# mlelarge/graph_neural_net

Hardware: AMD Instinct MI355X
Metric: graph-pairs/sec FGNN fwd+bwd, N=50 regular pairs (higher is better)
Workload: dtype f32

## Files before the change

### graph_neural_net_amd/_lib.py

```python
import ctypes as C
import os

import torch

_HERE = os.path.dirname(os.path.abspath(__file__))
LIB_PATH = os.environ.get('FGNN_LIB') or os.path.join(_HERE, 'libfgnn_hip.so')

FGNN_H = 32
FGNN_TILE = 32
FGNN_MAX_DEPTH = 3
FGNN_RANGE_WG = 256
FGNN_LSAP_MAX_N = 2048
FGNN_MAX_LEVELS = 64
FGNN_QAP_MAX_N = 256
FGNN_QAPW_MAX_N = 256
FGNN_SPECTRAL_MAX_N = 256
FGNN_SPECTRAL_MAX_POWERS = 8
FGNN_PLANTED_MAX_N = 256
FGNN_SCORE_SPLIT = 4

c_float_p = C.c_void_p


class Slab(C.Structure):
# ... 62 lines not shown
                ('s12tiles', C.c_void_p), ('s12_out', C.c_void_p), ('xbits', C.c_void_p), ('xdeg', C.c_void_p),
                ('ranges', C.c_void_p), ('cu_share', C.c_int)]


class Slab16(C.Structure):
    _fields_ = [('ptr', C.c_void_p), ('gstride', C.c_longlong), ('ldp', C.c_longlong), ('C', C.c_int),
                ('nrm', C.c_void_p), ('beta', C.c_void_p)]


class MlpFwd16Args(C.Structure):
    _fields_ = [('G', C.c_int), ('N', C.c_int), ('ldr', C.c_int), ('depth', C.c_int), ('nmlp', C.c_int),
                ('nvalid', C.c_void_p),
                ('a', Slab16), ('b', Slab16),
                ('z', C.c_void_p * 2), ('ldz', C.c_longlong),
                ('part', C.c_void_p * 2), ('cnt', C.c_void_p), ('packed', C.c_void_p), ('ranges', C.c_void_p)]


class MlpBwd16Args(C.Structure):
    _fields_ = [('G', C.c_int), ('N', C.c_int), ('ldr', C.c_int), ('depth', C.c_int),
                ('nvalid', C.c_void_p),
                ('a', Slab16), ('b', Slab16),
                ('dy', C.c_void_p), ('dgstride', C.c_longlong), ('ldd', C.c_longlong),
                ('z', C.c_void_p), ('zgstride', C.c_longlong), ('ldz', C.c_longlong),
                ('coef', C.c_void_p),
                ('dxa', C.c_void_p), ('dxa_gstride', C.c_longlong), ('dxa_ld', C.c_longlong),
                ('dxb', C.c_void_p), ('dxb_gstride', C.c_longlong), ('dxb_ld', C.c_longlong),
                ('accumulate_a', C.c_int), ('accumulate_b', C.c_int),
                ('wpart', C.c_void_p), ('s12part', C.c_void_p), ('packed', C.c_void_p), ('ranges', C.c_void_p)]


class GradJob(C.Structure):
    _fields_ = [('wpart', C.c_void_p), ('count', C.c_int), ('out', C.c_void_p), ('s12', C.c_void_p),
                ('nrm', C.c_void_p), ('dgn_w', C.c_void_p), ('dgn_b', C.c_void_p), ('rows', C.c_int), ('scale', C.c_float), ('scale_dev', C.c_void_p)]


class PackJob(C.Structure):
    _fields_ = [('kind', C.c_int), ('ca', C.c_int), ('cb', C.c_int), ('depth', C.c_int), ('nmlp', C.c_int),
                ('W', (C.c_void_p * FGNN_MAX_DEPTH) * 2), ('bias', (C.c_void_p * FGNN_MAX_DEPTH) * 2),
                ('out', C.c_void_p)]


class PairgenArgs(C.Structure):
    _fields_ = [('seed', C.c_ulonglong), ('first', C.c_longlong), ('B', C.c_int), ('N', C.c_int),
                ('family', C.c_int), ('noise_model', C.c_int), ('edge_density', C.c_double),
                ('thr_edge', C.c_ulonglong), ('thr_noise1', C.c_ulonglong), ('thr_noise2', C.c_ulonglong),
                ('thr_vertex', C.c_ulonglong), ('swaps_per_edge', C.c_int),
                ('bits1', C.c_void_p), ('bits2', C.c_void_p), ('nvalid', C.c_void_p)]


FGNN_GUARD_MAX_PARTS = 64
FGNN_GUARD_SKIP_NONFINITE = 1
FGNN_GUARD_NONFINITE = 1


class GuardRecord(C.Structure):
    _fields_ = [('max_norm', C.c_double), ('norm', C.c_double), ('coef', C.c_double),
                ('flags', C.c_int), ('skipped', C.c_int), ('arrivals', C.c_int), ('mode', C.c_int),
                ('partial', C.c_double * FGNN_GUARD_MAX_PARTS)]


class EvalRecord(C.Structure):
    _fields_ = [('ce_sum', C.c_double), ('nodes', C.c_longlong), ('correct_lsap', C.c_longlong), ('correct_max', C.c_longlong),
                ('pairs', C.c_longlong), ('steps', C.c_longlong)]


MAX_GRAD_JOBS = 16
MAX_PACK_JOBS = 24
_VP, _LL, _I, _F = C.c_void_p, C.c_longlong, C.c_int, C.c_float

_SIGNATURES = {
    'fgnn_last_error': [],
    'fgnn_version': [],
    'fgnn_tiles_per_graph': [_I],
    'fgnn_mlp_bwd_num_workgroups': [],
    'fgnn_pack_floats': [_I, _I, _I, _I, _I],
    'fgnn_pack_operands': [_VP, _I, _VP],
    'fgnn_mlp_fwd': [C.POINTER(MlpFwdArgs), _VP],
    'fgnn_pack_x3_floats': [_I, _I, _I, _I, _I],
    'fgnn_pack_x3_operands': [_VP, _I, _VP],
    'fgnn_mlp_fwd_x3': [C.POINTER(MlpFwdArgs), _VP],
    'fgnn_debug_mlp_fwd_masks': [C.POINTER(MlpFwdArgs), _VP, _VP, _VP],
    'fgnn_debug_mlp_fwd_x3_masks': [C.POINTER(MlpFwdArgs), _VP, _VP, _VP],
    'fgnn_debug_matmul_variant': [_I],
    'fgnn_gn_finalize': [_VP, _VP, _VP, _VP, _I, _I, _I, _F, _VP, _VP],
    'fgnn_gn_finalize2': [_VP, _VP, _VP, _VP, _VP, _VP, _I, _I, _I, _F, _VP, _VP, _VP],
    'fgnn_gn_plane_supported': [_I],
    'fgnn_gn_plane_fwd': [_VP, _LL, _LL, _VP, _VP, _VP, _I, _I, _I, _F, _VP, _LL, _LL, _VP, _VP],
    'fgnn_gn_plane_bwd': [_VP, _LL, _LL, _VP, _LL, _LL, _VP, _VP, _I, _I, _I, _VP, _LL, _LL, _VP, _VP, _VP, _VP],
    'fgnn_gn_stats': [_VP, _LL, _LL, _VP, _VP, _I, _I, _I, _F, _VP, _VP],
    'fgnn_gn_apply': [_VP, _LL, _LL, _VP, _VP, _VP, _I, _I, _I, _VP, _LL, _LL, _VP],
    'fgnn_ragged_tile_ranges': [_VP, _I, _I, _VP, _VP],
    'fgnn_ragged_tile_ranges_order': [_VP, _I, _I, _VP, _VP, _VP],
    'fgnn_ragged_tile_ranges16': [_VP, _I, _I, _I, _VP, _VP],
    'fgnn_conv1x1_dw_multi': [C.POINTER(DwJob), _I, _VP, _I, _I, _VP, _VP],
    'fgnn_conv_chain_supported': [_I, _I, C.POINTER(C.c_int)],
    'fgnn_conv_chain': [C.POINTER(ChainArgs), _VP],
    'fgnn_mlp64_supported': [_I, _I, _I],
    'fgnn_mlp64_num_workgroups': [],
    'fgnn_mlp64_param_count': [_I],
    'fgnn_mlp64_packed_floats': [_I],
    'fgnn_mlp64_pack': [_VP, _VP, _VP, _VP, _VP, _VP, _I, _VP, _VP],
    'fgnn_mlp64_pack_multi': [C.POINTER(Mlp64PackJob), _I, _VP],
    'fgnn_mlp64_fwd': [C.POINTER(Mlp64Args), _VP],
    'fgnn_mlp64_bwd': [C.POINTER(Mlp64Args), _VP],
    'fgnn_conv1x1': [_VP, _LL, _LL, _VP, _VP, _LL, _LL, _VP, _I, _VP, _I, _I, _I, _I, _VP, _LL, _LL, _VP],
    'fgnn_conv1x1_dw_chunks': [_I, _I],
    'fgnn_conv1x1_dw': [_VP, _LL, _LL, _VP, _VP, _LL, _LL, _VP, _I, _I, _I, _I, _VP, _VP],
    'fgnn_chan_matmul_fwd': [C.POINTER(Slab), C.POINTER(Slab), _VP, _I, _I, _VP, _LL, _LL, _VP],
    'fgnn_chan_matmul_fwd_ord': [C.POINTER(Slab), C.POINTER(Slab), _VP, _I, _I, _VP, _LL, _LL, _VP, _I, _VP],
    'fgnn_chan_matmul_fwd_fin_supported': [_I],
    'fgnn_chan_matmul_fwd_fin': [C.POINTER(Slab), C.POINTER(Slab), _VP, _VP, _VP, _VP, _VP, _F, _VP, _I, _I, _VP, _LL, _LL, _VP],
    'fgnn_chan_matmul_fwd_fin_ord': [C.POINTER(Slab), C.POINTER(Slab), _VP, _VP, _VP, _VP, _VP, _F, _VP, _I, _I, _VP, _LL, _LL, _VP, _I, _VP],
    'fgnn_colmax_fwd': [C.POINTER(Slab), _VP, _I, _I, _VP, _VP, _VP],
    'fgnn_colmax_fwd_fin_supported': [_I],
    'fgnn_colmax_fwd_fin': [C.POINTER(Slab), _VP, _VP, _VP, _F, _VP, _I, _I, _VP, _VP, _VP],
    'fgnn_score_ce_fwd': [_VP, _VP, _VP, _I, _I, _I, _VP, _VP, _VP, _VP],
    'fgnn_score_row_blocks': [_I, _I],
    'fgnn_score_ce_fwd_blocks': [_VP, _VP, _VP, _I, _I, _I, _I, _VP, _VP, _VP, _VP],
    'fgnn_score_ce_bwd': [_VP, _VP, _VP, _VP, _VP, _VP, _I, _I, _I, _VP, _VP, _VP],
    'fgnn_score_ce_fwd_blocks_labels': [_VP, _VP, _VP, _VP, _I, _I, _I, _I, _VP, _VP, _VP, _VP],
    'fgnn_score_ce_bwd_labels': [_VP, _VP, _VP, _VP, _VP, _VP, _VP, _I, _I, _I, _VP, _VP, _VP],
    'fgnn_ce_fwd_labels': [_VP, _VP, _VP, _I, _I, _VP, _VP, _VP],
    'fgnn_ce_bwd_labels': [_VP, _VP, _VP, _VP, _VP, _I, _I, _VP, _VP],
    'fgnn_inv_node_count': [_VP, _I, _VP, _VP],
    'fgnn_score_bwd': [_VP, _VP, _VP, _VP, _I, _I, _I, _VP, _VP, _VP],
    'fgnn_ce_fwd': [_VP, _VP, _I, _I, _VP, _VP, _VP],
    'fgnn_ce_bwd': [_VP, _VP, _VP, _VP, _I, _I, _VP, _VP],
    'fgnn_colmax_bwd': [_VP, _VP, _VP, _I, _I, _I, _VP, _LL, _LL, C.POINTER(Slab), _VP, _VP],
    'fgnn_gn_bwd_stats': [_VP, _LL, _LL, _VP, _LL, _LL, _VP, _VP, _I, _I, _I, _VP, _VP],
    'fgnn_gn_bwd_coef': [_VP, _VP, _VP, _I, _I, _I, _VP, _VP, _VP, _VP],
    'fgnn_gn_bwd_coef_tiles': [_VP, _VP, _VP, _I, _I, _I, _VP, _VP, _VP],
    'fgnn_grad_finalize': [_VP, _I, _I, _I, _I, _VP],
    'fgnn_gn_bwd_apply': [_VP, _LL, _LL, _VP, _LL, _LL, _VP, _VP, _I, _I, _I, _VP, _LL, _LL, _VP],
    'fgnn_mlp_bwd': [C.POINTER(MlpBwdArgs), _VP],
    'fgnn_mlp_bwd_x3': [C.POINTER(MlpBwdArgs), _VP],
    'fgnn_mlp_bwd_pair': [C.POINTER(MlpBwdArgs), C.POINTER(MlpBwdArgs), _VP],
    'fgnn_mlp_bwd_t16': [C.POINTER(MlpBwdArgs), _VP],
    'fgnn_mlp_bwd_t16_supported': [C.POINTER(MlpBwdArgs)],
    'fgnn_mlp_bwd_pair_t16': [C.POINTER(MlpBwdArgs), C.POINTER(MlpBwdArgs), _VP],
    'fgnn_mlp_bwd_pair_x3': [C.POINTER(MlpBwdArgs), C.POINTER(MlpBwdArgs), _VP],
    'fgnn_block1_struct_supported': [_I, _I, _I],
    'fgnn_block1_struct_table_floats': [_I],
    'fgnn_block1_struct_ws_floats': [_I, _I],
    'fgnn_block1_struct_rows': [_I, _I],
    'fgnn_block1_struct_fwd': [_VP, _VP, _I, _I, _VP, _VP, _VP, _VP, _VP, C.c_float, _VP, _VP, _VP, _LL, _LL, _VP, _VP, _VP, _VP, _VP, _VP, _VP],
    'fgnn_block1_struct_bwd': [_VP, _VP, _I, _I, _VP, _VP, _VP, _VP, _VP, _VP, _VP, _VP, _LL, _LL, _VP, _VP, _VP, _VP, _VP, _VP],
    'fgnn_block1_struct_fwd_pack': [_VP, _VP, _I, _I, _VP, _VP, _VP, _VP, _VP, C.c_float, _VP, _VP, _VP, _LL, _LL, _VP, _VP, _VP, _VP, _VP, _VP, _VP, _I, _VP],
    'fgnn_block1_struct_fwd16_pack': [_VP, _VP, _I, _I, _I, _VP, _VP, _VP, _VP, _VP, C.c_float, _VP, _VP, _VP, _LL, _LL, _VP, _VP, _VP, _VP, _VP, _VP, _VP, _I, _VP],
    'fgnn_block1_struct_fwd16': [_VP, _VP, _I, _I, _I, _VP, _VP, _VP, _VP, _VP, C.c_float, _VP, _VP, _VP, _LL, _LL, _VP, _VP, _VP, _VP, _VP, _VP, _VP],
    'fgnn_block1_struct_bwd16': [_VP, _VP, _I, _I, _I, _VP, _VP, _VP, _VP, _VP, _VP, _VP, _VP, _LL, _LL, _VP, _VP, _VP, _VP, _VP, _VP],
    'fgnn_mlp_bwd_coef_tiles_supported': [_I, _I],
    'fgnn_mlp_param_count': [_I, _I],
    'fgnn_reduce_partials': [_VP, _I, _I, _VP, _VP],
    'fgnn_chan_matmul_bwd': [C.POINTER(Slab), C.POINTER(Slab), _VP, _LL, _LL, _VP, _I, _I, _VP, _VP, _LL, _LL, _VP, _VP, _VP],
    'fgnn_chan_matmul_bwd_ord': [C.POINTER(Slab), C.POINTER(Slab), _VP, _LL, _LL, _VP, _I, _I, _VP, _VP, _LL, _LL, _VP, _VP, _VP, _I, _VP],
    'fgnn_sum_scale': [_VP, _I, _I, _F, _VP, _VP],
    'fgnn_adam_step': [_VP, _VP, _VP, _VP, _I, C.c_double, C.c_double, C.c_double, C.c_double, _I, C.c_double, _VP],
    'fgnn_adam_step_dev': [_VP, _VP, _VP, _VP, _I, _VP, _VP, _VP],
    'fgnn_grad_guard': [_VP, _I, _VP, _VP, _VP],
    'fgnn_adam_step_guarded': [_VP, _VP, _VP, _VP, _I, _VP, _VP, _VP, _VP],
    'fgnn_expand_adjacency': [_VP, _VP, _I, _I, _VP, _VP],
    'fgnn_pack_adjacency': [_VP, _VP, _I, _I, _VP, _VP, _VP],
    'fgnn_pack_adjacency_ld': [_VP, _VP, _I, _I, _I, _VP, _VP, _VP],
    'fgnn_pack_adjacency_pair': [_VP, _VP, _VP, _VP, _I, _I, _I, _VP, _VP, _VP, _VP, _VP],
    'fgnn_adjacency_degree': [_VP, _VP, _I, _I, _VP, _VP],
    'fgnn_accuracy_max': [_VP, _VP, _I, _I, _VP, _VP],
# ... 147 lines not shown
```

### graph_neural_net_amd/csrc/matmul.hip

```cpp
#include "fgnn_common.h"
#include "fgnn_norm.h"

namespace {

constexpr int TM = 64;
constexpr int LDS_LD = 65;

struct NormRec {
    float mean, a, beta;
    bool on;
};

DEVI NormRec norm_of(const fgnn_slab &s, int g, int c) {
    NormRec r;
    r.on = s.nrm != nullptr;
    if (r.on) {
        const float4 n = reinterpret_cast<const float4 *>(s.nrm)[(long long)g * s.C + c];
        r.mean = n.x;
        r.a = n.y;
        r.beta = s.beta ? s.beta[c] : 0.f;
    } else {
        r.mean = 0.f;
        r.a = 1.f;
        r.beta = 0.f;
// ... 121 lines not shown
    if (s12a && live) {
        const int col = col0 + 32 * qj + j;
#pragma unroll
        for (int r = 0; r < 16; ++r) {
            const int row = row0 + 32 * qi + ch_of(r, h);
            if (row < nv && col < nv) {
                sa1 += acc[r];
                sa2 += acc[r] * (A[(long long)row * N + col] - na.mean);
            }
        }
    }

#pragma unroll
    for (int r = 0; r < 16; ++r) acc[r] = 0.f;
    for (int i0 = 0; i0 < N; i0 += TM) {
        __syncthreads();
        stage_tile(Xs, A, N, nv, i0, row0, na, tid);
        stage_tile(Ds, D, N, nv, i0, col0, none, tid);
        __syncthreads();
        if (live) {
            const int kmax = (N - i0 < TM ? N - i0 : TM);
            const float *ap = Xs + h * LDS_LD + 32 * qi + j;
            const float *bp = Ds + h * LDS_LD + 32 * qj + j;
            for (int k = 0; k < kmax; k += 2) acc = mfma32(ap[k * LDS_LD], bp[k * LDS_LD], acc);
        }
    }
    if (live) store_quadrant(OB, N, row0 + 32 * qi, col0 + 32 * qj, acc, lane);
    if (s12a) {
        if (live) {
            const int col = col0 + 32 * qj + j;
#pragma unroll
            for (int r = 0; r < 16; ++r) {
                const int row = row0 + 32 * qi + ch_of(r, h);
                if (row < nv && col < nv) {
                    sb1 += acc[r];
                    sb2 += acc[r] * (B[(long long)row * N + col] - nb.mean);
                }
            }
        }
        sa1 = wave_sum(sa1);
        sa2 = wave_sum(sa2);
        sb1 = wave_sum(sb1);
        sb2 = wave_sum(sb2);
        if (lane == 0) {
            red[wave][0] = sa1;
            red[wave][1] = sa2;
            red[wave][2] = sb1;
            red[wave][3] = sb2;
        }
        __syncthreads();
        if (tid < 4) {
            const float v = (red[0][tid] + red[1][tid]) + (red[2][tid] + red[3][tid]);
            float *dst = (tid < 2 ? s12a : s12b) + (long long)gc * 2 + (tid & 1);
            *dst = v;
        }
    }
}

template <bool WANT_U>
DEVI void load_tile_regs(float (&v)[16], float (&u)[16], const float *mat, int N, int nv, const NormRec &nr, int tid) {
#pragma unroll
    for (int k = 0; k < 16; ++k) {
        const int e = tid + 256 * k;
        const int r = e >> 6, c = e & 63;
        const bool ok = r < nv && c < nv;
        const float x = mat[ok ? r * N + c : 0];
        const float d = x - nr.mean;
        v[k] = ok ? (nr.on ? d * nr.a + nr.beta : x) : 0.f;
        if (WANT_U) u[k] = ok ? d : 0.f;
    }
}
DEVI void store_tile_lds(float *lds, const float (&v)[16], int tid) {
#pragma unroll
    for (int k = 0; k < 16; ++k) {
        const int e = tid + 256 * k;
        lds[(e >> 6) * LDS_LD + (e & 63)] = v[k];
    }
}
DEVI void frag_to_lds(float *lds, int row0, int col0, const f32x16 &acc, int lane) {
    const int j = lane & 31, h = lane >> 5;
#pragma unroll
    for (int r = 0; r < 16; ++r) lds[(row0 + ch_of(r, h)) * LDS_LD + col0 + j] = acc[r];
}
template <bool WANT_S>
DEVI void tile_to_global(const View &ov, int mat_off4, const float *lds, int N, const float (&u)[16], float &s1,
                         float &s2, int tid) {
    const int c = tid & 63, r0 = __builtin_amdgcn_readfirstlane(tid >> 6);
    const int voff = c < N ? (r0 * N + c) * 4 : OOB_OFF;
    const float *lp = lds + r0 * LDS_LD + c;
#pragma unroll
    for (int k = 0; k < 16; ++k) {
        const float t = lp[4 * k * LDS_LD];
        buf_store(t, ov, r0 + 4 * k < N ? voff : OOB_OFF, mat_off4 + k * 16 * N);
        if (WANT_S) {
            s1 += t;
            s2 += t * u[k];
        }
    }
}

DEVI void load_tile_raw(float (&x)[16], const View &v, int mat_off4, int N, int nv, int tid) {
    const int c = tid & 63, r0 = __builtin_amdgcn_readfirstlane(tid >> 6);
    const int voff = c < nv ? (r0 * N + c) * 4 : OOB_OFF;
#pragma unroll
    for (int k = 0; k < 16; ++k) {
        const int r = r0 + 4 * k;
        x[k] = buf_load(v, r < nv ? voff : OOB_OFF, mat_off4 + k * 16 * N);
    }
}
template <bool WANT_U>
DEVI void finish_tile(float (&v)[16], float (&u)[16], const float (&x)[16], int nv, const NormRec &nr, int tid) {
#pragma unroll
    for (int k = 0; k < 16; ++k) {
        const int e = tid + 256 * k;
        const int r = e >> 6, c = e & 63;
        const bool ok = r < nv && c < nv;
        const float d = x[k] - nr.mean;
        v[k] = ok ? (nr.on ? d * nr.a + nr.beta : x[k]) : 0.f;
        if (WANT_U) u[k] = ok ? d : 0.f;
    }
}

struct FinArgs {
    const float *part_a, *part_b, *cnt, *gw_a, *gw_b;
    float *nrm_a, *nrm_b;
    float eps;
    int tpg;
};
template <bool FIN>
__global__ __launch_bounds__(256, 4) void chan_matmul_fwd1_kernel(const fgnn_slab ya, const fgnn_slab yb,
                                                               const int *nvalid, int N, int M, float *out,
                                                               long long ogstride, long long ldo, const FinArgs F) {
    __shared__ float As[TM * LDS_LD];
    __shared__ float Bs[TM * LDS_LD];
    __shared__ float4 fin_rec[2];
    const int C = ya.C;
    const int tid = threadIdx.x, lane = tid & 63, wave = tid >> 6;
    const int qi = wave >> 1, qj = wave & 1;
    const int j = lane & 31, h = lane >> 5;
    float xa[16], xb[16], dummy[16];
    const int G = M / C;
    const View vA = make_view(ya.ptr, ya.gstride, ya.ldp, G), vB = make_view(yb.ptr, yb.gstride, yb.ldp, G);
    const View vO = make_view(out, ogstride, ldo, G);
    const int gc = blockIdx.x;
    {
        const int g = gc / C, c = gc - g * C;
        const int nv = nvalid_of(nvalid, g, N);
        TilePartials tp;
        if (FIN && wave < 2) tp = finalize_load(wave ? F.part_b : F.part_a, F.cnt, g, c, C, F.tpg, lane);
        load_tile_raw(xa, vA, g * vA.gs4 + c * vA.ld4, N, nv, tid);
        load_tile_raw(xb, vB, g * vB.gs4 + c * vB.ld4, N, nv, tid);
        NormRec na, nb;
        if (FIN) {
            if (wave < 2) {
                const float4 r = finalize_reduce(tp, (float)nv, (wave ? F.gw_b : F.gw_a) ? (wave ? F.gw_b : F.gw_a)[c] : 1.f, F.eps);
                if (lane == 0) {
                    fin_rec[wave] = r;
                    reinterpret_cast<float4 *>(wave ? F.nrm_b : F.nrm_a)[gc] = r;
                }
            }
            __syncthreads();
            const float4 ra = fin_rec[0], rb = fin_rec[1];
            na.on = true; na.mean = ra.x; na.a = ra.y; na.beta = ya.beta ? ya.beta[c] : 0.f;
            nb.on = true; nb.mean = rb.x; nb.a = rb.y; nb.beta = yb.beta ? yb.beta[c] : 0.f;
        } else {
            na = norm_of(ya, g, c);
            nb = norm_of(yb, g, c);
        }
        const int o_off = g * vO.gs4 + c * vO.ld4;
        {
            float va[16], vb[16];
            finish_tile<false>(va, dummy, xa, nv, na, tid);
            finish_tile<false>(vb, dummy, xb, nv, nb, tid);
            store_tile_lds(As, va, tid);
            store_tile_lds(Bs, vb, tid);
// ... 24 lines not shown
    __shared__ float Ds[TM * LDS_LD];
    __shared__ float red[4][4];
    const int C = ya.C;
    const int tid = threadIdx.x, lane = tid & 63, wave = tid >> 6;
    const int qi = wave >> 1, qj = wave & 1;
    const int j = lane & 31, h = lane >> 5;
    NormRec none;
    none.on = false; none.mean = 0.f; none.a = 1.f; none.beta = 0.f;
    float xa[16], xb[16], xd[16], dummy[16];
    const int G = M / C;
    const View vA = make_view(ya.ptr, ya.gstride, ya.ldp, G), vB = make_view(yb.ptr, yb.gstride, yb.ldp, G);
    const View vD = make_view(dm, dmg, ldm, G);
    const View vOA = make_view(da, ogstride, ldo, G), vOB = make_view(db, ogstride, ldo, G);
    const int gc = blockIdx.x;
    {
        const int g = gc / C, c = gc - g * C;
        const int nv = nvalid_of(nvalid, g, N);
        load_tile_raw(xa, vA, g * vA.gs4 + c * vA.ld4, N, nv, tid);
        load_tile_raw(xb, vB, g * vB.gs4 + c * vB.ld4, N, nv, tid);
        load_tile_raw(xd, vD, g * vD.gs4 + c * vD.ld4, N, nv, tid);
        const NormRec na = norm_of(ya, g, c), nb = norm_of(yb, g, c);
        const int o_off = g * vOA.gs4 + c * vOA.ld4;
        float ua[16], ub[16], va[16];
        finish_tile<true>(va, ua, xa, nv, na, tid);
        {
            float vb[16], vd[16];
            finish_tile<true>(vb, ub, xb, nv, nb, tid);
            finish_tile<false>(vd, dummy, xd, nv, none, tid);
            store_tile_lds(Bs, vb, tid);
            store_tile_lds(Ds, vd, tid);
        }
        __syncthreads();
        const bool live = 32 * qi < N && 32 * qj < N;
        f32x16 accA, accB;
#pragma unroll
        for (int r = 0; r < 16; ++r) {
            accA[r] = 0.f;
            accB[r] = 0.f;
        }
        if (live) {
            const float *ap = Ds + (32 * qi + j) * LDS_LD + h;
            const float *bp = Bs + (32 * qj + j) * LDS_LD + h;
            for (int k = 0; k < N; k += 2) accA = mfma32(ap[k], bp[k], accA);
        }
        __syncthreads();
        store_tile_lds(Bs, va, tid);
        __syncthreads();
        if (live) {
            const float *ap = Bs + h * LDS_LD + 32 * qi + j;
            const float *bp = Ds + h * LDS_LD + 32 * qj + j;
            for (int k = 0; k < N; k += 2) accB = mfma32(ap[k * LDS_LD], bp[k * LDS_LD], accB);
        }
        __syncthreads();
        frag_to_lds(Ds, 32 * qi, 32 * qj, accA, lane);
        frag_to_lds(Bs, 32 * qi, 32 * qj, accB, lane);
        __syncthreads();
        float sa1 = 0.f, sa2 = 0.f, sb1 = 0.f, sb2 = 0.f;
        if (s12a) {
            tile_to_global<true>(vOA, o_off, Ds, N, ua, sa1, sa2, tid);
            tile_to_global<true>(vOB, o_off, Bs, N, ub, sb1, sb2, tid);
            sa1 = wave_sum(sa1);
            sa2 = wave_sum(sa2);
            sb1 = wave_sum(sb1);
            sb2 = wave_sum(sb2);
            if (lane == 0) {
                red[wave][0] = sa1;
                red[wave][1] = sa2;
                red[wave][2] = sb1;
                red[wave][3] = sb2;
            }
            __syncthreads();
            if (tid < 4) {
                const float v = (red[0][tid] + red[1][tid]) + (red[2][tid] + red[3][tid]);
                float *dst = (tid < 2 ? s12a : s12b) + (long long)gc * 2 + (tid & 1);
                *dst = v;
            }
        } else {
            tile_to_global<false>(vOA, o_off, Ds, N, dummy, sa1, sa2, tid);
            tile_to_global<false>(vOB, o_off, Bs, N, dummy, sb1, sb2, tid);
        }
    }
}


int g_mm_wave_variant = 1;
inline bool mm_wave_variant() { return (g_mm_wave_variant & 1) != 0; }
inline bool mm_narrow() { return (g_mm_wave_variant & 8) != 0; }
constexpr int WLD = 68;
constexpr int W_WAVES = 2;

DEVI rsrc_t mat_rsrc(const float *p, int bytes) {
    return __builtin_amdgcn_make_buffer_rsrc(const_cast<float *>(p), 0, bytes, 0x00020000);
}
DEVI float rsrc_load(rsrc_t r, int voff, int soff) {
    return __builtin_bit_cast(float, __builtin_amdgcn_raw_buffer_load_b32(r, voff, soff, 0));
}
DEVI void rsrc_store(float x, rsrc_t r, int voff, int soff) {
    __builtin_amdgcn_raw_buffer_store_b32(__builtin_bit_cast(unsigned, x), r, voff, soff, 0);
}

template <int KQ>
DEVI void wave_rows_load(float (&x)[8 * KQ], rsrc_t r, int N, int voff) {
#pragma unroll
    for (int i = 0; i < 8 * KQ; ++i) x[i] = rsrc_load(r, voff, i < N ? i * N * 4 : 0);
}
template <int KQ>
DEVI void wave_rows_stage(float *T, const float (&x)[8 * KQ], float mean, float a_eff, float b_eff, int nv, int N, int lane) {
    if (nv < N) {
#pragma unroll
        for (int i = 0; i < 8 * KQ; ++i) {
            const float v = (x[i] - mean) * a_eff + b_eff;
            T[i * WLD + lane] = i < nv ? v : 0.f;
        }
    } else {
#pragma unroll
        for (int i = 0; i < 8 * KQ; ++i) T[i * WLD + lane] = (x[i] - mean) * a_eff + b_eff;
    }
}

template <int KQ, bool FIN>
__global__ __launch_bounds__(64 * W_WAVES, 2) void chan_matmul_fwd_w_kernel(const fgnn_slab ya, const fgnn_slab yb,
                                                                           const int *nvalid, int N, int M, float *out,
                                                                           long long ogstride, long long ldo,
                                                                           const FinArgs F) {
    constexpr int KH = 4 * KQ;
    constexpr bool TWO = KQ > 4;
    constexpr int NB = TWO ? 2 : 1;
    __shared__ __attribute__((aligned(16))) float lds[W_WAVES * 32 * NB * WLD];
    const int lane = threadIdx.x & 63, wv = __builtin_amdgcn_readfirstlane(threadIdx.x >> 6);
    const int gc = xcd_swizzle(blockIdx.x, gridDim.x) * W_WAVES + wv;
    if (gc >= M) return;
    const int C = ya.C;
    const int g = gc / C, c = gc - g * C;
    const int nv = __builtin_amdgcn_readfirstlane(nvalid_of(nvalid, g, N));
    const int j = lane & 31, h = lane >> 5;
    float *As = lds + wv * (32 * NB * WLD);
    const rsrc_t rA = mat_rsrc(ya.ptr + (long long)g * ya.gstride + (long long)c * ya.ldp, nv * N * 4);
    const rsrc_t rB = mat_rsrc(yb.ptr + (long long)g * yb.gstride + (long long)c * yb.ldp, nv * N * 4);
    const rsrc_t rO = mat_rsrc(out + (long long)g * ogstride + (long long)c * ldo, N * N * 4);

    TilePartials ta, tb;
    if (FIN) {
        ta = finalize_load(F.part_a, F.cnt, g, c, C, F.tpg, lane);
        tb = finalize_load(F.part_b, F.cnt, g, c, C, F.tpg, lane);
    }
    float xa[8 * KQ], xb[NB][KH];
    wave_rows_load<KQ>(xa, rA, N, lane < nv ? lane * 4 : OOB_OFF);
    int voffB[NB];
#pragma unroll
    for (int cb = 0; cb < NB; ++cb) {
        const int col = 32 * cb + j;
        voffB[cb] = col < nv ? (h * N + col) * 4 : OOB_OFF;
    }
#pragma unroll
    for (int s = 0; s < KH; ++s)
#pragma unroll
        for (int cb = 0; cb < NB; ++cb) xb[cb][s] = rsrc_load(rB, voffB[cb] + s * 2 * N * 4, 0);
    float meanA, aA, meanB, aB;
    if (FIN) {
        const float4 ra = finalize_reduce(ta, (float)nv, F.gw_a ? F.gw_a[c] : 1.f, F.eps);
        const float4 rb = finalize_reduce(tb, (float)nv, F.gw_b ? F.gw_b[c] : 1.f, F.eps);
        if (lane == 0) {
            reinterpret_cast<float4 *>(F.nrm_a)[gc] = ra;
            reinterpret_cast<float4 *>(F.nrm_b)[gc] = rb;
        }
        meanA = ra.x; aA = ra.y; meanB = rb.x; aB = rb.y;
    } else {
        const NormRec na = norm_of(ya, g, c), nb = norm_of(yb, g, c);
// ... 518 lines not shown
        sa2 = wave_sum(sa2);
        sb1 = wave_sum(sb1);
        sb2 = wave_sum(sb2);
        if (lane == 0) {
            red[wv][0] = sa1;
            red[wv][1] = sa2;
            red[wv][2] = sb1;
            red[wv][3] = sb2;
        }
        __syncthreads();
        if (tid < 4 && (tid < 2 ? do_a : do_b)) {
            float v = 0.f;
#pragma unroll
            for (int w = 0; w < BIG_NW; ++w) v += red[w][tid];
            float *dst = (tid < 2 ? s12a : s12b) + (long long)gc * 2 + (tid & 1);
            *dst = v;
        }
    }
}

inline bool big_path(int N) { return N > TM && N <= 256; }

}

template <int MT, bool FIN>
static void launch_fwd_big(const fgnn_slab *ya, const fgnn_slab *yb, const int *nvalid, int N, int G, float *out, long long ogstride,
                           long long ldo, const int *order, const FinArgs &F, int fill, hipStream_t st) {
    static LdsAttrCache attr_cache;
    (void)fgnn_raise_lds(attr_cache, (const void *)chan_matmul_fwd_big_kernel<MT, FIN>, BigCfg<MT>::LDS_BYTES);
    hipLaunchKernelGGL((chan_matmul_fwd_big_kernel<MT, FIN>), dim3(G * ya->C), dim3(BIG_THREADS), BigCfg<MT>::LDS_BYTES, st, *ya, *yb, nvalid, N, G, out,
                       ogstride, ldo, order, F, fill);
}

extern "C" int fgnn_chan_matmul_fwd(const fgnn_slab *ya, const fgnn_slab *yb, const int *nvalid, int G, int N,
                                    float *out, long long ogstride, long long ldo, void *stream) {
    return fgnn_chan_matmul_fwd_ord(ya, yb, nvalid, G, N, out, ogstride, ldo, nullptr, 0, stream);
}

extern "C" int fgnn_chan_matmul_fwd_ord(const fgnn_slab *ya, const fgnn_slab *yb, const int *nvalid, int G, int N,
                                        float *out, long long ogstride, long long ldo, const int *order, int fill, void *stream) {
    FGNN_CHECK(!order || nvalid, "fgnn_chan_matmul_fwd_ord: an order needs the nvalid it was derived from");
    FGNN_CHECK(ya && yb && out && ya->ptr && yb->ptr, "fgnn_chan_matmul_fwd: null argument");
    FGNN_CHECK(ya->C == yb->C && ya->C > 0 && G > 0 && N > 0, "fgnn_chan_matmul_fwd: bad shapes");
    FGNN_CHECK((long long)G * ya->C <= 65535 * 1024ll, "fgnn_chan_matmul_fwd: G*C too large");
    const int t = (N + TM - 1) / TM;
    if (t == 1) {
        FGNN_CHECK((long long)G * ya->gstride < 0x7fffffffll / 4 && (long long)G * yb->gstride < 0x7fffffffll / 4,
                   "fgnn_chan_matmul_fwd: a tensor exceeds 2 GiB (32-bit buffer addressing); split the batch");
        FGNN_CHECK((long long)G * ogstride < 0x7fffffffll / 4, "fgnn_chan_matmul_fwd: output exceeds 2 GiB");
        const int M = G * ya->C;
        if (mm_wave_variant()) {
            launch_fwd_w<false>(ya, yb, nvalid, N, M, out, ogstride, ldo, FinArgs{}, (hipStream_t)stream);
            FGNN_LAUNCH_CHECK();
            return 0;
        }
        hipLaunchKernelGGL(chan_matmul_fwd1_kernel<false>, dim3(M), dim3(256), 0, (hipStream_t)stream, *ya, *yb, nvalid,
                           N, M, out, ogstride, ldo, FinArgs{});
        FGNN_LAUNCH_CHECK();
        return 0;
    }
    if (big_path(N)) {
        FGNN_CHECK((long long)G * ya->gstride < 0x7fffffffll / 4 && (long long)G * yb->gstride < 0x7fffffffll / 4 &&
                   (long long)G * ogstride < 0x7fffffffll / 4,
                   "fgnn_chan_matmul_fwd: a tensor exceeds 2 GiB (32-bit buffer addressing); split the batch");
        if (N <= 128) launch_fwd_big<4, false>(ya, yb, nvalid, N, G, out, ogstride, ldo, order, FinArgs{}, fill, (hipStream_t)stream);
        else launch_fwd_big<8, false>(ya, yb, nvalid, N, G, out, ogstride, ldo, order, FinArgs{}, fill, (hipStream_t)stream);
        FGNN_LAUNCH_CHECK();
        return 0;
    }
    hipLaunchKernelGGL(chan_matmul_fwd_kernel, dim3(t, t, G * ya->C), dim3(256), 0, (hipStream_t)stream, *ya, *yb,
                       nvalid, N, out, ogstride, ldo);
    FGNN_LAUNCH_CHECK();
    return 0;
}

extern "C" int fgnn_chan_matmul_fwd_fin_supported(int N) { return (N <= TM || big_path(N)) ? 1 : 0; }

extern "C" int fgnn_debug_matmul_variant(int wave_per_matrix) {
    FGNN_CHECK((wave_per_matrix & ~9) == 0, "fgnn_debug_matmul_variant: bits 0 and 3 only (got %d)", wave_per_matrix);
    g_mm_wave_variant = wave_per_matrix;
    return 0;
}

extern "C" int fgnn_chan_matmul_fwd_fin(const fgnn_slab *ya, const fgnn_slab *yb, const float *part_a, const float *part_b,
                                        const float *cnt, const float *gn_weight_a, const float *gn_weight_b, float eps,
                                        const int *nvalid, int G, int N, float *out, long long ogstride, long long ldo,
                                        void *stream) {
    return fgnn_chan_matmul_fwd_fin_ord(ya, yb, part_a, part_b, cnt, gn_weight_a, gn_weight_b, eps, nvalid, G, N, out, ogstride, ldo, nullptr, 0, stream);
}

extern "C" int fgnn_chan_matmul_fwd_fin_ord(const fgnn_slab *ya, const fgnn_slab *yb, const float *part_a, const float *part_b,
                                            const float *cnt, const float *gn_weight_a, const float *gn_weight_b, float eps,
                                            const int *nvalid, int G, int N, float *out, long long ogstride, long long ldo,
                                            const int *order, int fill, void *stream) {
    FGNN_CHECK(!order || nvalid, "fgnn_chan_matmul_fwd_fin_ord: an order needs the nvalid it was derived from");
    FGNN_CHECK(ya && yb && out && ya->ptr && yb->ptr && part_a && part_b && cnt, "fgnn_chan_matmul_fwd_fin: null argument");
    FGNN_CHECK(ya->nrm && yb->nrm, "fgnn_chan_matmul_fwd_fin: the slabs must carry the record buffers to fill");
    FGNN_CHECK(ya->C == yb->C && ya->C > 0 && G > 0 && N > 0, "fgnn_chan_matmul_fwd_fin: bad shapes");
    FGNN_CHECK(N <= TM || big_path(N), "fgnn_chan_matmul_fwd_fin: N=%d > 256 (use fgnn_gn_finalize2 + fgnn_chan_matmul_fwd)", N);
    FGNN_CHECK((long long)G * ya->gstride < 0x7fffffffll / 4 && (long long)G * yb->gstride < 0x7fffffffll / 4 &&
               (long long)G * ogstride < 0x7fffffffll / 4,
               "fgnn_chan_matmul_fwd_fin: a tensor exceeds 2 GiB (32-bit buffer addressing); split the batch");
    const int M = G * ya->C;
    FinArgs F = {part_a, part_b, cnt, gn_weight_a, gn_weight_b, const_cast<float *>(ya->nrm), const_cast<float *>(yb->nrm), eps,
                 fgnn_tiles_per_graph(N)};
    if (big_path(N)) {
        if (N <= 128) launch_fwd_big<4, true>(ya, yb, nvalid, N, G, out, ogstride, ldo, order, F, fill, (hipStream_t)stream);
        else launch_fwd_big<8, true>(ya, yb, nvalid, N, G, out, ogstride, ldo, order, F, fill, (hipStream_t)stream);
        FGNN_LAUNCH_CHECK();
        return 0;
    }
    if (mm_wave_variant()) {
        launch_fwd_w<true>(ya, yb, nvalid, N, M, out, ogstride, ldo, F, (hipStream_t)stream);
        FGNN_LAUNCH_CHECK();
        return 0;
    }
    hipLaunchKernelGGL(chan_matmul_fwd1_kernel<true>, dim3(M), dim3(256), 0, (hipStream_t)stream, *ya, *yb, nvalid, N, M, out,
                       ogstride, ldo, F);
    FGNN_LAUNCH_CHECK();
    return 0;
}

extern "C" int fgnn_chan_matmul_bwd(const fgnn_slab *ya, const fgnn_slab *yb, const float *dm, long long dmgstride,
                                    long long ldm, const int *nvalid, int G, int N, float *da, float *db,
                                    long long ogstride, long long ldo, float *s12a, float *s12b, void *stream) {
    return fgnn_chan_matmul_bwd_ord(ya, yb, dm, dmgstride, ldm, nvalid, G, N, da, db, ogstride, ldo, s12a, s12b, nullptr,
                                    0, stream);
}

extern "C" int fgnn_chan_matmul_bwd_ord(const fgnn_slab *ya, const fgnn_slab *yb, const float *dm, long long dmgstride,
                                        long long ldm, const int *nvalid, int G, int N, float *da, float *db,
                                        long long ogstride, long long ldo, float *s12a, float *s12b, const int *order,
                                        int fill, void *stream) {
    FGNN_CHECK(!order || nvalid, "fgnn_chan_matmul_bwd_ord: an order needs the nvalid it was derived from");
    FGNN_CHECK(ya && yb && dm && da && db && ya->ptr && yb->ptr, "fgnn_chan_matmul_bwd: null argument");
    FGNN_CHECK(ya->C == yb->C && ya->C > 0 && G > 0 && N > 0, "fgnn_chan_matmul_bwd: bad shapes");
    FGNN_CHECK((s12a == nullptr) == (s12b == nullptr), "fgnn_chan_matmul_bwd: s12a and s12b come together");
    FGNN_CHECK(!s12a || (ya->nrm && yb->nrm), "fgnn_chan_matmul_bwd: s12 outputs need normalised slabs");
    const int t = (N + TM - 1) / TM;
    const bool fused = s12a && t == 1;
    if (t == 1) {
        FGNN_CHECK((long long)G * ya->gstride < 0x7fffffffll / 4 && (long long)G * yb->gstride < 0x7fffffffll / 4 &&
                   (long long)G * dmgstride < 0x7fffffffll / 4,
                   "fgnn_chan_matmul_bwd: a tensor exceeds 2 GiB (32-bit buffer addressing); split the batch");
        FGNN_CHECK((long long)G * ogstride < 0x7fffffffll / 4, "fgnn_chan_matmul_bwd: output exceeds 2 GiB");
        const int M = G * ya->C;
        hipLaunchKernelGGL(chan_matmul_bwd1_kernel, dim3(M), dim3(256), 0, (hipStream_t)stream, *ya, *yb, dm,
                           dmgstride, ldm, nvalid, N, M, da, db, ogstride, ldo, s12a, s12b);
        FGNN_LAUNCH_CHECK();
        return 0;
    }
    if (big_path(N)) {
        FGNN_CHECK((long long)G * ya->gstride < 0x7fffffffll / 4 && (long long)G * yb->gstride < 0x7fffffffll / 4 &&
                   (long long)G * dmgstride < 0x7fffffffll / 4 && (long long)G * ogstride < 0x7fffffffll / 4,
                   "fgnn_chan_matmul_bwd: a tensor exceeds 2 GiB (32-bit buffer addressing); split the batch");
#define FGNN_BIG_BWD(MT)                                                                                              \
    {                                                                                                                 \
        static LdsAttrCache attr_cache;                                                                           \
        (void)fgnn_raise_lds(attr_cache, (const void *)chan_matmul_bwd_big_kernel<MT>, BigCfg<MT>::LDS_BYTES);                   \
        hipLaunchKernelGGL(chan_matmul_bwd_big_kernel<MT>, dim3(G * ya->C * (split ? 2 : 1)), dim3(BIG_THREADS),      \
                           BigCfg<MT>::LDS_BYTES, (hipStream_t)stream, *ya, *yb, dm, dmgstride, ldm, nvalid, N, G, da, \
                           db, ogstride, ldo, s12a, s12b, order, split, fill);                                            \
    }
        const int split = (order && (long long)G * ya->C <= BIG_SPLIT_MAX_MATRICES) ? 1 : 0;
        if (N <= 128) FGNN_BIG_BWD(4)
        else FGNN_BIG_BWD(8)
#undef FGNN_BIG_BWD
        FGNN_LAUNCH_CHECK();
        return 0;
    }
    hipLaunchKernelGGL(chan_matmul_bwd_kernel, dim3(t, t, G * ya->C), dim3(256), 0, (hipStream_t)stream, *ya, *yb, dm,
                       dmgstride, ldm, nvalid, N, da, db, ogstride, ldo, fused ? s12a : nullptr, fused ? s12b : nullptr);
    FGNN_LAUNCH_CHECK();
    if (s12a && !fused) {
        int rc = fgnn_gn_bwd_stats(da, ogstride, ldo, ya->ptr, ya->gstride, ya->ldp, ya->nrm, nvalid, G, ya->C, N, s12a, stream);
        if (rc) return rc;
        rc = fgnn_gn_bwd_stats(db, ogstride, ldo, yb->ptr, yb->gstride, yb->ldp, yb->nrm, nvalid, G, yb->C, N, s12b, stream);
        if (rc) return rc;
    }
    return 0;
}
```

### include/fgnn_hip.h

```cpp
#ifndef FGNN_HIP_H
#define FGNN_HIP_H

#ifdef __cplusplus
extern "C" {
#endif

#define FGNN_H 32
#define FGNN_TILE 32
#define FGNN_MAX_DEPTH 3

typedef struct {
    const float *ptr;
    long long gstride;
    long long ldp;
    int C;
    const float *nrm;
    const float *beta;
} fgnn_slab;

const char *fgnn_last_error(void);
int fgnn_version(void);
int fgnn_tiles_per_graph(int N);
int fgnn_mlp_bwd_num_workgroups(void);

// ... 404 lines not shown
    int family, noise_model;
    double edge_density;
    unsigned long long thr_edge;
    unsigned long long thr_noise1;
    unsigned long long thr_noise2;
    unsigned long long thr_vertex;
    int swaps_per_edge;
    unsigned *bits1, *bits2;
    int *nvalid;
} fgnn_pairgen_args;
int fgnn_pairgen_supported(int N, int family, int noise_model);
int fgnn_pairgen(const fgnn_pairgen_args *args, void *stream);
int fgnn_pairgen_indexed(const fgnn_pairgen_args *args, const long long *index, void *stream);
#define FGNN_MAX_LEVELS 64
int fgnn_pairgen_levels(const fgnn_pairgen_args *args, const long long *index ,
                        const unsigned long long *level_thr , int K, const int *level , void *stream);

#define FGNN_EPOCH_ROUNDS 8
#define FGNN_EPOCH_STREAM 6
#define FGNN_EPOCH_MAX_LOG2_M 40
int fgnn_epoch_index(unsigned long long seed, unsigned long long epoch, long long M, long long first_pos, long long count,
                     long long *out, void *stream);

#define FGNN_PLANTED_STREAM 7
#define FGNN_PLANTED_MAX_N 256
int fgnn_planted_perm(unsigned long long seed, long long first, const long long *index , const int *nvalid ,
                      int B, int N, int *labels, void *stream);
int fgnn_relabel_bits(const unsigned *in, const int *labels, const int *nvalid, int B, int N, unsigned *out, void *stream);
int fgnn_relabel_dense(const float *in, const int *labels, const int *nvalid, int B, int C, int ld, int NL, float *out, void *stream);
int fgnn_count_matches(const int *assign, const int *labels, const int *nvalid, int B, int N, int *correct, void *stream);
int fgnn_accuracy_max_labels(const float *scores, const int *labels, const int *nvalid, int B, int N, int *correct, void *stream);

#define FGNN_QAP_MAX_N 256
int fgnn_qap_objective(const unsigned *bits1, const unsigned *bits2, const int *assign, const int *nvalid, int B, int N, int *qap,
                       int *planted, int *na, int *nb, void *stream);
int fgnn_qap_improve_cost(const unsigned *bits1, const unsigned *bits2, const int *assign, const int *nvalid, int B, int N, float *cost,
                          long long bstride, int ld, void *stream);
long long fgnn_greedy_qap_ws_bytes(int B, int N);
int fgnn_greedy_qap(const unsigned *bits1, const unsigned *bits2, const int *assign0, const int *nvalid, int B, int N, int T, void *ws,
                    long long ws_bytes, int *s_best2, int *acc_best, int *t_best, int *perm_best , void *stream);
int fgnn_greedy_qap_labels(const unsigned *bits1, const unsigned *bits2, const int *assign0, const int *labels, const int *nvalid, int B,
                           int N, int T, void *ws, long long ws_bytes, int *s_best2, int *acc_best, int *t_best,
                           int *perm_best , void *stream);

#define FGNN_QAPW_MAX_N 256
int fgnn_qapw_objective(const float *a1, const float *a2, long long gstride, int ld, const int *assign, const int *nvalid, int B, int N,
                        float *qap, float *trace, float *planted, float *na, float *nb, void *stream);
int fgnn_qapw_improve_cost(const float *a1, const float *a2, long long gstride, int ld, const int *assign, const int *nvalid, int B, int N,
                           float *cost, long long bstride, int cost_ld, void *stream);
long long fgnn_greedy_qapw_ws_bytes(int B, int N);
int fgnn_greedy_qapw(const float *a1, const float *a2, long long gstride, int ld, const int *assign0, const int *nvalid, int B, int N, int T,
                     void *ws, long long ws_bytes, float *s_best, int *acc_best, int *t_best, int *perm_best ,
                     void *stream);
int fgnn_greedy_qapw_labels(const float *a1, const float *a2, long long gstride, int ld, const int *assign0, const int *labels,
                            const int *nvalid, int B, int N, int T, void *ws, long long ws_bytes, float *s_best, int *acc_best,
                            int *t_best, int *perm_best , void *stream);

#define FGNN_SPECTRAL_MAX_N 256
#define FGNN_SPECTRAL_MAX_POWERS 8
int fgnn_spectral_features(const unsigned *bits, const int *nvalid, int G, int N, int n_powers, float *out, int Nout, void *stream);

typedef struct {
    double ce_sum;
    long long nodes;
    long long correct_lsap;
    long long correct_max;
    long long pairs;
    long long steps;
} fgnn_eval_record;
int fgnn_eval_pairs(const float *scores, const int *nvalid , const int *labels , int B, int N, float *cost,
                    long long cost_bstride, int cost_ld, float *row_ce, int *row_hit, void *stream);
int fgnn_eval_pairs_labels(const float *scores, const int *nvalid , const int *labels, int B, int N, float *cost,
                           long long cost_bstride, int cost_ld, float *row_ce, int *row_hit, void *stream);
int fgnn_eval_fold(const float *row_ce, const int *row_hit, const int *correct_lsap , const int *nvalid ,
                   int B, int N, int live, double *pair_ce , int *pair_max , fgnn_eval_record *meter,
                   void *stream);
int fgnn_eval_fold_bins(const float *row_ce, const int *row_hit, const int *correct_lsap , const int *nvalid ,
                        int B, int N, int live, const int *bin , int K, double *pair_ce ,
                        int *pair_max , fgnn_eval_record *records , void *stream);

int fgnn_debug_mlp_fwd_masks(const fgnn_mlp_fwd_args *args, unsigned *masks0, unsigned *masks1 , void *stream);
int fgnn_debug_mlp_fwd_x3_masks(const fgnn_mlp_fwd_args *args, unsigned *masks0, unsigned *masks1, void *stream);
int fgnn_debug_matmul_variant(int wave_per_matrix);

#ifdef __cplusplus
}
#endif
#endif
```

Baseline: 42470.

## Add MFMA-based small-N channel matmul backward kernel as default path

New measurement: 42620 (median of 6 runs). No clear change (+0.4%).

```diff
diff --git a/graph_neural_net_amd/_lib.py b/graph_neural_net_amd/_lib.py
--- a/graph_neural_net_amd/_lib.py
+++ b/graph_neural_net_amd/_lib.py
@@ -168,6 +168,7 @@
     'fgnn_debug_mlp_fwd_masks': [C.POINTER(MlpFwdArgs), _VP, _VP, _VP],
     'fgnn_debug_mlp_fwd_x3_masks': [C.POINTER(MlpFwdArgs), _VP, _VP, _VP],
     'fgnn_debug_matmul_variant': [_I],
+    'fgnn_debug_matmul_bwd_variant': [_I],
     'fgnn_gn_finalize': [_VP, _VP, _VP, _VP, _I, _I, _I, _F, _VP, _VP],
     'fgnn_gn_finalize2': [_VP, _VP, _VP, _VP, _VP, _VP, _I, _I, _I, _F, _VP, _VP, _VP],
     'fgnn_gn_plane_supported': [_I],
diff --git a/graph_neural_net_amd/csrc/matmul.hip b/graph_neural_net_amd/csrc/matmul.hip
--- a/graph_neural_net_amd/csrc/matmul.hip
+++ b/graph_neural_net_amd/csrc/matmul.hip
@@ -227,15 +227,15 @@
 #pragma unroll
     for (int r = 0; r < 16; ++r) lds[(row0 + ch_of(r, h)) * LDS_LD + col0 + j] = acc[r];
 }
-template <bool WANT_S>
+template <bool WANT_S, int LD = LDS_LD>
 DEVI void tile_to_global(const View &ov, int mat_off4, const float *lds, int N, const float (&u)[16], float &s1,
                          float &s2, int tid) {
     const int c = tid & 63, r0 = __builtin_amdgcn_readfirstlane(tid >> 6);
     const int voff = c < N ? (r0 * N + c) * 4 : OOB_OFF;
-    const float *lp = lds + r0 * LDS_LD + c;
+    const float *lp = lds + r0 * LD + c;
 #pragma unroll
     for (int k = 0; k < 16; ++k) {
-        const float t = lp[4 * k * LDS_LD];
+        const float t = lp[4 * k * LD];
         buf_store(t, ov, r0 + 4 * k < N ? voff : OOB_OFF, mat_off4 + k * 16 * N);
         if (WANT_S) {
             s1 += t;
@@ -426,8 +426,138 @@
     }
 }
 
+constexpr int QLD = 68;
+constexpr int QOUT = 64;
+
+DEVI void stage_rows(float *T, const float (&v)[16], int r0, int p) {
+    float *tp = T + r0 * QLD + p;
+#pragma unroll
+    for (int k = 0; k < 16; ++k) tp[4 * k * QLD] = v[k];
+}
+
+__global__ __launch_bounds__(256, 4) void chan_matmul_bwd1q_kernel(const fgnn_slab ya, const fgnn_slab yb,
+                                                                const float *dm, long long dmg, long long ldm,
+                                                                const int *nvalid, int N, int M, float *da, float *db,
+                                                                long long ogstride, long long ldo, float *s12a,
+                                                                float *s12b) {
+    __shared__ __attribute__((aligned(16))) float Bs[TM * QLD];
+    __shared__ __attribute__((aligned(16))) float Ds[TM * QLD];
+    __shared__ float red[4][4];
+    const int C = ya.C;
+    const int tid = threadIdx.x, lane = tid & 63, wave = tid >> 6;
+    const int qi = wave >> 1, qj = wave & 1;
+    const int j = lane & 31, h = lane >> 5;
+    const int r0 = __builtin_amdgcn_readfirstlane(tid >> 6);
+    float xa[16], xb[16], xd[16], dummy[16];
+    const int G = M / C;
+    const View vA = make_view(ya.ptr, ya.gstride, ya.ldp, G), vB = make_view(yb.ptr, yb.gstride, yb.ldp, G);
+    const View vD = make_view(dm, dmg, ldm, G);
+    const View vOA = make_view(da, ogstride, ldo, G), vOB = make_view(db, ogstride, ldo, G);
+    const int gc = blockIdx.x;
+    const int g = gc / C, c = gc - g * C;
+    const int nv = nvalid_of(nvalid, g, N);
+    load_tile_raw(xb, vB, g * vB.gs4 + c * vB.ld4, N, nv, tid);
+    load_tile_raw(xd, vD, g * vD.gs4 + c * vD.ld4, N, nv, tid);
+    load_tile_raw(xa, vA, g * vA.gs4 + c * vA.ld4, N, nv, tid);
+    const NormRec na = norm_of(ya, g, c), nb = norm_of(yb, g, c);
+    const int o_off = g * vOA.gs4 + c * vOA.ld4;
+    const int pcol = (lane & 1) * 32 + (lane >> 1);
+    {
+        float vb[16];
+#pragma unroll
+        for (int k = 0; k < 16; ++k) {
+            xb[k] = xb[k] - nb.mean;
+            const float v = xb[k] * nb.a + nb.beta;
+            vb[k] = r0 + 4 * k < nv ? v : 0.f;
+        }
+        stage_rows(Bs, vb, r0, pcol);
+        stage_rows(Ds, xd, r0, pcol);
+    }
+    __syncthreads();
+    const int nsteps = (N + 1) >> 1;
+    f32x16 accA, accB;
+#pragma unroll
+    for (int r = 0; r < 16; ++r) {
+        accA[r] = 0.f;
+        accB[r] = 0.f;
+    }
+    if (32 * qi < N && 32 * qj < N) {
+        const float *ap = Ds + (32 * qi + j) * QLD + 32 * h;
+        const float *bp = Bs + (32 * qj + j) * QLD + 32 * h;
+        int s = 0;
+        for (; s + 4 <= nsteps; s += 4) {
+            const float4 a = *reinterpret_cast<const float4 *>(ap + s), b = *reinterpret_cast<const float4 *>(bp + s);
+            accA = mfma32(a.x, b.x, accA);
+            accA = mfma32(a.y, b.y, accA);
+            accA = mfma32(a.z, b.z, accA);
+            accA = mfma32(a.w, b.w, accA);
+        }
+        for (; s < nsteps; ++s) accA = mfma32(ap[s], bp[s], accA);
+    }
+    __syncthreads();
+    {
+        const bool okc = lane < nv;
+        const float a_eff = okc ? na.a : 0.f, b_eff = okc ? na.beta : 0.f;
+        float va[16];
+#pragma unroll
+        for (int k = 0; k < 16; ++k) {
+            xa[k] = xa[k] - na.mean;
+            va[k] = xa[k] * a_eff + b_eff;
+        }
+        stage_rows(Bs, va, r0, lane);
+    }
+    __syncthreads();
+    if (32 * qi < N && qj < N) {
+        const float *ap = Bs + h * QLD + 32 * qi + j;
+        const float *bp = Ds + h * QLD + 32 * qj + j;
+        int s = 0;
+        for (; s + 4 <= nsteps; s += 4) {
+            const float a0 = ap[(2 * s) * QLD], a1 = ap[(2 * s + 2) * QLD], a2 = ap[(2 * s + 4) * QLD], a3 = ap[(2 * s + 6) * QLD];
+            const float b0 = bp[(2 * s) * QLD], b1 = bp[(2 * s + 2) * QLD], b2 = bp[(2 * s + 4) * QLD], b3 = bp[(2 * s + 6) * QLD];
+            accB = mfma32(a0, b0, accB);
+            accB = mfma32(a1, b1, accB);
+            accB = mfma32(a2, b2, accB);
+            accB = mfma32(a3, b3, accB);
+        }
+        for (; s < nsteps; ++s) accB = mfma32(ap[(2 * s) * QLD], bp[(2 * s) * QLD], accB);
+    }
+    __syncthreads();
+#pragma unroll
+    for (int r = 0; r < 16; ++r) {
+        const int row = 32 * qi + ch_of(r, h);
+        Ds[row * QOUT + 32 * qj + j] = accA[r];
+        Bs[row * QOUT + 2 * j + qj] = accB[r];
+    }
+    __syncthreads();
+    float sa1 = 0.f, sa2 = 0.f, sb1 = 0.f, sb2 = 0.f;
+    if (s12a) {
+        tile_to_global<true, QOUT>(vOA, o_off, Ds, N, xa, sa1, sa2, tid);
+        tile_to_global<true, QOUT>(vOB, o_off, Bs, N, xb, sb1, sb2, tid);
+        sa1 = wave_sum(sa1);
+        sa2 = wave_sum(sa2);
+        sb1 = wave_sum(sb1);
+        sb2 = wave_sum(sb2);
+        if (lane == 0) {
+            red[wave][0] = sa1;
+            red[wave][1] = sa2;
+            red[wave][2] = sb1;
+            red[wave][3] = sb2;
+        }
+        __syncthreads();
+        if (tid < 4) {
+            const float v = (red[0][tid] + red[1][tid]) + (red[2][tid] + red[3][tid]);
+            float *dst = (tid < 2 ? s12a : s12b) + (long long)gc * 2 + (tid & 1);
+            *dst = v;
+        }
+    } else {
+        tile_to_global<false, QOUT>(vOA, o_off, Ds, N, dummy, sa1, sa2, tid);
+        tile_to_global<false, QOUT>(vOB, o_off, Bs, N, dummy, sb1, sb2, tid);
+    }
+}
+
 
 int g_mm_wave_variant = 1;
+int g_mm_bwd_variant = 0;
 inline bool mm_wave_variant() { return (g_mm_wave_variant & 1) != 0; }
 inline bool mm_narrow() { return (g_mm_wave_variant & 8) != 0; }
 constexpr int WLD = 68;
@@ -1112,6 +1242,12 @@
     return 0;
 }
 
+extern "C" int fgnn_debug_matmul_bwd_variant(int first_form) {
+    FGNN_CHECK(first_form == 0 || first_form == 1, "fgnn_debug_matmul_bwd_variant: 0 or 1 (got %d)", first_form);
+    g_mm_bwd_variant = first_form;
+    return 0;
+}
+
 extern "C" int fgnn_chan_matmul_fwd_fin(const fgnn_slab *ya, const fgnn_slab *yb, const float *part_a, const float *part_b,
                                         const float *cnt, const float *gn_weight_a, const float *gn_weight_b, float eps,
                                         const int *nvalid, int G, int N, float *out, long long ogstride, long long ldo,
@@ -1175,8 +1311,12 @@
                    "fgnn_chan_matmul_bwd: a tensor exceeds 2 GiB (32-bit buffer addressing); split the batch");
         FGNN_CHECK((long long)G * ogstride < 0x7fffffffll / 4, "fgnn_chan_matmul_bwd: output exceeds 2 GiB");
         const int M = G * ya->C;
-        hipLaunchKernelGGL(chan_matmul_bwd1_kernel, dim3(M), dim3(256), 0, (hipStream_t)stream, *ya, *yb, dm,
-                           dmgstride, ldm, nvalid, N, M, da, db, ogstride, ldo, s12a, s12b);
+        if (g_mm_bwd_variant == 1)
+            hipLaunchKernelGGL(chan_matmul_bwd1_kernel, dim3(M), dim3(256), 0, (hipStream_t)stream, *ya, *yb, dm,
+                               dmgstride, ldm, nvalid, N, M, da, db, ogstride, ldo, s12a, s12b);
+        else
+            hipLaunchKernelGGL(chan_matmul_bwd1q_kernel, dim3(M), dim3(256), 0, (hipStream_t)stream, *ya, *yb, dm,
+                               dmgstride, ldm, nvalid, N, M, da, db, ogstride, ldo, s12a, s12b);
         FGNN_LAUNCH_CHECK();
         return 0;
     }
diff --git a/include/fgnn_hip.h b/include/fgnn_hip.h
--- a/include/fgnn_hip.h
+++ b/include/fgnn_hip.h
@@ -510,6 +510,7 @@
 int fgnn_debug_mlp_fwd_masks(const fgnn_mlp_fwd_args *args, unsigned *masks0, unsigned *masks1 , void *stream);
 int fgnn_debug_mlp_fwd_x3_masks(const fgnn_mlp_fwd_args *args, unsigned *masks0, unsigned *masks1, void *stream);
 int fgnn_debug_matmul_variant(int wave_per_matrix);
+int fgnn_debug_matmul_bwd_variant(int first_form);
 
 #ifdef __cplusplus
 }
```
